# ZYM-PKU/UDiffText

Measured on AMD Instinct MI355X. Metric: 512x512 50-step denoised images/sec (UDiffText hot path: conditioner + 50 CFG Euler steps + VAE decode), higher is better.
Workload: dtype bf16; 1 GPU; 512x512, 50 Euler/DDIM(eta 0) steps, CFG 5.0, 9-char labels, noise_iters 0; global batch 4 per step sharded over 1 GPU(s) = 4 images per GPU in micro-batches of 4: every UNet call runs ONE batch of 4 (8 samples with CFG); 3 such batch(es) in flight per GPU on separate launch streams; BASELINE.json configs[1]; global_batch=4, weights=synthetic (name-keyed recipe), 1361.2 M parameters, launch=hipGraph replay of the sampler steps, in_flight=3, batches_per_unet_call=1

## Files before the change

udifftext_amd/csrc/gemm.hip:

```cpp
#include "common.h"
#include <stdio.h>
#include <stdlib.h>
#include <string.h>
#include <atomic>
#include <cmath>

hipError_t udt_lean_launch_gemm(int cfg, const void* lparams, int smem, int G, int geglu, int ln, hipStream_t s);
hipError_t udt_lean_launch_conv3(const void* c3params, hipStream_t s);

namespace {
#include "tile_common.h"

struct GemmParams {
  const uint16_t* a;
  const uint16_t* a2;
  const uint16_t* w;
  const uint16_t* zero;
  const float* bias;
  const uint16_t* res;
  const float* rowvec;
  void* out;
  const float* colscale;
  const float* in_scsh;
  float* colstats;
// ... 821 lines not shown
  t.G = round_workgroups(units);
  int nb = g_n_block.load(std::memory_order_relaxed);
  if (nb <= 0) nb = (t.tiles_m <= 8) ? t.tiles_n : 8;
  if (nb > t.tiles_n) nb = t.tiles_n;
  t.n_block = nb;
  return true;
}

size_t lean_workspace(const LeanPlan& t) {
  return t.splitk > 1 ? G8_HEADER_BYTES + (size_t)t.tiles * t.splitk * t.bm * t.bn * sizeof(float) : 0;
}

std::atomic<int> g_lean_conv{-1};
std::atomic<int> g_wide_conv{-2};
int wide_conv_mode() {
  int v = g_wide_conv.load(std::memory_order_relaxed);
  if (v == -2) {
    const char* e = getenv("UDT_WIDE_CONV");
    v = e ? atoi(e) : -1;
    g_wide_conv.store(v, std::memory_order_relaxed);
  }
  return v;
}
#ifdef UDT_MEASURE
std::atomic<int> g_lconv_dbg{0};
#endif

std::atomic<int> g_wide_lanes_eff{-2};
double wide_lanes_eff() {
  int v = g_wide_lanes_eff.load(std::memory_order_relaxed);
  if (v == -2) {
    const char* e = getenv("UDT_WIDE_LANES_EFF");
    v = e ? atoi(e) : 70;
    g_wide_lanes_eff.store(v, std::memory_order_relaxed);
  }
  return v / 100.0;
}

int conv_chunk_slices(long long tiles, int slots, int chunks, int knob) {
  long long sk = 1;
  if (tiles <= 1023) {
    if (knob > 1) { sk = knob; if (sk > chunks) sk = chunks; }
    else if (knob < 0 && tiles * 2 <= slots && chunks >= 10) { sk = slots / tiles; if (sk > chunks / 4) sk = chunks / 4; }
    if (sk < 1) sk = 1;
  }
  return (int)sk;
// ... 13 lines not shown
  if (d->N < 128 || d->N % 8 != 0 || d->C1 <= 0 || d->C1 % 64 != 0) return false;
  if (d->upsample != 0 && d->upsample != 1 && d->upsample != 2) return false;
  const bool phase = d->upsample == 2, ups = d->upsample == 1;
  const int nph = phase ? 4 : 1;
  if (d->Hout != (d->Hin << (d->upsample ? 1 : 0)) || d->Wout != (d->Win << (d->upsample ? 1 : 0))) return false;
  if (phase && d->ldw > 0 && d->ldw < 4 * d->C1) return false;
  const int Ht = phase ? d->Hin : d->Hout, Wt = phase ? d->Win : d->Wout;
  c.bn = 128; c.wgm = 2;
  bool wide = false;
  int wide_slots = device_cus();
  {
    const int wm = wide_conv_mode();
    if (wm != 0 && !ups && d->N % 160 == 0 && Wt % 16 == 0 && Ht % 16 == 0) {
      const int cus = device_cus(), share = d->cu_share > 1 ? d->cu_share : 1;
      wide_slots = cus / share > 0 ? cus / share : 1;
      const long long wt = (long long)(d->M / 256) * (d->N / 160);
      const long long sk = conv_chunk_slices(wt, wide_slots, d->C1 / 64, lean_splitk_knob());
      const long long units = wt * sk;
      const long long rounds = (units + cus - 1) / cus;
      const double eff = units > cus ? (double)units / (double)(rounds * cus) : ((double)units * share >= cus ? 1.0 : (double)units * share / cus);
      wide = (wm > 0) || (sk <= 2 && eff >= ((share >= 3 && share_of(d) >= 3) ? wide_lanes_eff() : 0.85));
    }
  }
  if (wide) { c.geo = phase ? 6 : 3; c.tw = 16; c.th = 16; c.bn = 160; c.wgm = 4; }
  else if (Wt % 16 == 0 && Ht % 8 == 0) { c.geo = ups ? 2 : phase ? 4 : 0; c.tw = 16; c.th = 8; }
  else if (!ups && Wt % 8 == 0 && Ht % 8 == 0) { c.geo = phase ? 5 : 1; c.tw = 8; c.th = 8; }
  else return false;
  if (d->ldo % 8 != 0 || (d->residual && d->ldr % 8 != 0)) return false;
  const long long ldw = d->ldw > 0 ? d->ldw : (phase ? 4LL * d->C1 : (long long)d->K);
  if (ldw % 8 != 0) return false;
  c.w_phase = phase ? (d->stride_w > 0 ? d->stride_w : (long long)d->N * ldw) : 0;
  if (phase && (c.w_phase < (long long)d->N * ldw || c.w_phase % 8 != 0)) return false;
  if ((long long)d->M * d->C1 * 2 >= (1LL << 31) || (long long)d->N * ldw * 2 >= (1LL << 31)) return false;
  if ((reinterpret_cast<uintptr_t>(d->out) | reinterpret_cast<uintptr_t>(d->residual) | reinterpret_cast<uintptr_t>(d->bias) |
       reinterpret_cast<uintptr_t>(d->rowvec)) & 15) return false;
  if (d->rowvec && ((d->ld_rowvec > 0 ? d->ld_rowvec : d->N) % 4 != 0)) return false;
  c.dbg = 0;
#ifdef UDT_MEASURE
  c.dbg = g_lconv_dbg.load(std::memory_order_relaxed);
#endif
  c.N = d->N; c.C = d->C1; c.H = d->Hin; c.W = d->Win; c.B = d->M / (d->Hout * d->Wout);
  c.ldw = (int)ldw; c.ldo = d->ldo; c.ldr = d->ldr; c.ldrv = d->ld_rowvec > 0 ? d->ld_rowvec : d->N;
  c.alpha = d->alpha;
  c.tiles_x = Wt / c.tw; c.tiles_y = Ht / c.th;
  c.tiles_m = c.B * c.tiles_x * c.tiles_y;
  c.tiles_n = (d->N + c.bn - 1) / c.bn;
  c.tiles = c.tiles_m * c.tiles_n;
// ... 38 lines not shown
  LeanPlan lt;
  if (lean_plan(d, lt, true)) {
    rows = lt.stats_rows;
    slots = lt.tiles_m * (lt.bm / lt.stats_rows);
    return true;
  }
  return false;
}
}

extern "C" int udt_debug_set(const char* key, int32_t value) {
  if (!key) return UDT_ERR_BAD_ARG;
  if (!strcmp(key, "n_block")) { g_n_block.store(value); return UDT_OK; }
  if (!strcmp(key, "rows_epi")) { g_rows_epi.store(value ? 1 : 0); return UDT_OK; }
  if (!strcmp(key, "lean")) { g_lean.store(value < 0 ? -2 : value); return UDT_OK; }
  if (!strcmp(key, "rowres")) { g_rowres.store(value < 0 ? 1 : (value ? 1 : 0)); return UDT_OK; }
  if (!strcmp(key, "wide_lanes_eff")) { g_wide_lanes_eff.store(value < 0 ? -2 : value); return UDT_OK; }
  if (!strcmp(key, "conv_n4")) { g_conv_n4.store(value < 0 ? -2 : (value ? 1 : 0)); return UDT_OK; }
  if (!strcmp(key, "lean256_lanes")) { g_lean256_lanes.store(value < 0 ? -2 : (value ? 1 : 0)); return UDT_OK; }
  if (!strcmp(key, "lean_splitk")) { g_lean_splitk.store(value); return UDT_OK; }
  if (!strcmp(key, "share_splitk")) { g_share_splitk.store(value < 0 ? -2 : (value ? 1 : 0)); return UDT_OK; }
  if (!strcmp(key, "lean_conv")) { g_lean_conv.store(value < 0 ? -1 : (value ? 1 : 0)); return UDT_OK; }
  if (!strcmp(key, "wide_conv")) { g_wide_conv.store(value < 0 ? -1 : (value ? 1 : 0)); return UDT_OK; }
#ifdef UDT_MEASURE
  if (!strcmp(key, "lconv_dbg")) { g_lconv_dbg.store(value); return UDT_OK; }
  static const struct { const char* k; int bit; } bits[] = {{"no_xchg", 28}, {"no_epi", 27}, {"no_store", 26}, {"no_res", 25},
                                                            {"no_bias", 24}, {"no_fast", 22}};
  for (const auto& b : bits)
    if (!strcmp(key, b.k)) {
      int cur = g_dbg_bits.load();
      g_dbg_bits.store((cur & ~(1 << b.bit)) | (value ? (1 << b.bit) : 0));
      return UDT_OK;
    }
#endif
  return UDT_ERR_BAD_ARG;
}

extern "C" int udt_check_async_error(void* workspace, size_t workspace_bytes, void* stream) {
  if (!workspace || workspace_bytes < G8_HEADER_BYTES) return UDT_ERR_BAD_ARG;
  hipStream_t s = reinterpret_cast<hipStream_t>(stream);
  int err = 0;
  hipError_t e = hipMemcpyAsync(&err, reinterpret_cast<int*>(workspace) + 1023, sizeof(int), hipMemcpyDeviceToHost, s);
  if (e == hipSuccess) e = hipStreamSynchronize(s);
  if (e != hipSuccess) return udt_set_hip_error(e);
  if (err == 0) return UDT_OK;
  e = hipMemsetAsync(workspace, 0, G8_HEADER_BYTES, s);
// ... 215 lines not shown
        udt_prof_tag(profl.rec, tag);
      }
      const bool geglu = (d->flags & UDT_GEMM_GEGLU) != 0, ln = d->ln_colsum != nullptr;
      hipError_t el;
      el = udt_lean_launch_gemm(lt.cfg, &lp, lt.smem, lt.G, geglu ? 1 : 0, ln ? 1 : 0, s);
      if (el != hipSuccess) return udt_set_hip_error(el);
      return UDT_OK;
    }
  }
  if (d->ln_colsum) return UDT_ERR_BAD_ARG;
  {
    lg::C3Params c3;
    if (lean_conv_plan(d, c3, d->colstats != nullptr)) {
      c3.colstats = d->colstats;
      c3.a = p.a; c3.w = p.w; c3.bias = p.bias; c3.res = p.res; c3.rowvec = p.rowvec; c3.out = reinterpret_cast<uint16_t*>(d->out);
      if (c3.splitk > 1) {
        if (!workspace || workspace_bytes < lean_conv_workspace(c3)) return UDT_ERR_WORKSPACE;
        c3.counters = reinterpret_cast<int*>(workspace);
        c3.slabs = reinterpret_cast<float*>(reinterpret_cast<char*>(workspace) + G8_HEADER_BYTES);
      }
      UdtProfScope profc(cls, s);
      if (profc.rec) {
        char tag[96];
        snprintf(tag, sizeof(tag), "%s%s M=%d N=%d K=%d %dx%d tile=%dx%d units=%d splitk=%d nb=%d%s", (c3.geo == 3 || c3.geo == 6) ? "wconv3" : "lconv3",
                 (d->upsample && c3.geo != 6) ? "+up" : "", d->M, d->N, d->K,
                 d->Hin, d->Win, c3.tw, c3.th, c3.tiles * lean_conv_phases(c3) * c3.splitk, c3.splitk, c3.n_block,
                 d->upsample == 2 ? " up4" : "");
        udt_prof_tag(profc.rec, tag);
      }
      const hipError_t ec = udt_lean_launch_conv3(&c3, s);
      if (ec != hipSuccess) return udt_set_hip_error(ec);
      return UDT_OK;
    }
  }
  {
    c3p::CParams cp;
    if (conv3p_geometry(d, cp.geo, d->in_scsh != nullptr)) {
      const TilePlan t3 = plan_tiles3p(d, cp.geo);
      p.tiles_m = t3.tiles_m; p.tiles_n = t3.tiles_n; p.tiles_per_batch = t3.tiles_m * t3.tiles_n;
      {
        const double patch = (double)cp.geo.prows_img * cp.geo.NI * cp.geo.C * 2.0;
        const double wtile = 9.0 * t3.bn * cp.geo.C * 2.0;
        const double S = (double)(t3.tiles < t3.G ? t3.tiles : t3.G) / 8.0;
        int nb = (int)(std::sqrt((S < 1.0 ? 1.0 : S) * patch / wtile) + 0.5);
        if (nb < 1) nb = 1;
        if (nb > t3.tiles_n) nb = t3.tiles_n;
        p.n_block = nb;
      }
      p.n_ktiles = t3.nkt;
// ... 111 lines not shown
```

udifftext_amd/csrc/lean.hip:

```cpp
#include "common.h"
#include <stdio.h>
#include <stdlib.h>
#include <atomic>

namespace {
#include "tile_common.h"
#include "lean_params.h"
#include "lean.h"
#include "wide.h"
#include "rowres.h"

template <int NW, int WGM, int WGN, int TM, int TN, int NST, int TMB = TM>
hipError_t launch_lean(const lg::LParams& lp, int smem, int G, bool geglu, bool ln, hipStream_t s) {
  static AttrOnce once[5];
  const void* fn;
  const bool stats = lp.colstats != nullptr;
  if constexpr (NW == 4 && NST == 2) {
    if (stats) {
      fn = (const void*)lg::lgemm_kernel<NW, WGM, WGN, TM, TN, NST, false, false, TMB, true>;
      hipError_t e = once[4].ensure(fn, smem);
      if (e != hipSuccess) return e;
      void* args[] = {const_cast<lg::LParams*>(&lp)};
      return hipLaunchKernel(fn, dim3(G), dim3(NW * 64), args, smem, s);
    }
// ... 28 lines not shown
  }
  if (geglu) return (ln && emit && !stats) ? launch_lean_mx8_k<true, true, false, true, true>(lp, smem, G, s) : hipErrorInvalidValue;
  if (ln) return stats ? hipErrorInvalidValue
                 : emit ? launch_lean_mx8_k<false, true, false, true, true>(lp, smem, G, s)
                        : launch_lean_mx8_k<false, true, false, true, false>(lp, smem, G, s);
  if (stats) return emit ? hipErrorInvalidValue : launch_lean_mx8_k<false, false, true, true, false>(lp, smem, G, s);
  return emit ? launch_lean_mx8_k<false, false, false, true, true>(lp, smem, G, s) : launch_lean_mx8_k<false, false, false, true, false>(lp, smem, G, s);
}

template <int TW, int TH, bool UPS, bool STATS, bool PHASE>
hipError_t launch_lconv3s(const lg::C3Params& c3, hipStream_t s) {
  static AttrOnce once;
  constexpr int smem = lg::C3Geo<TW, TH, UPS>::SMEM;
  hipError_t e = once.ensure(reinterpret_cast<const void*>(lg::lconv3_kernel<TW, TH, UPS, STATS, PHASE>), smem);
  if (e != hipSuccess) return e;
  hipLaunchKernelGGL((lg::lconv3_kernel<TW, TH, UPS, STATS, PHASE>), dim3(c3.G), dim3(256), smem, s, c3);
  return hipGetLastError();
}
template <int TW, int TH, bool UPS, bool PHASE = false>
hipError_t launch_lconv3(const lg::C3Params& c3, hipStream_t s) {
  return c3.colstats ? launch_lconv3s<TW, TH, UPS, true, PHASE>(c3, s) : launch_lconv3s<TW, TH, UPS, false, PHASE>(c3, s);
}

template <bool STATS, bool PHASE>
hipError_t launch_wconv3s(const lg::C3Params& c3, hipStream_t s) {
  static AttrOnce once;
  constexpr int smem = wd::WGeo::SMEM;
  hipError_t e = once.ensure(reinterpret_cast<const void*>(wd::wconv3_kernel<STATS, PHASE>), smem);
  if (e != hipSuccess) return e;
  hipLaunchKernelGGL((wd::wconv3_kernel<STATS, PHASE>), dim3(c3.G), dim3(256), smem, s, c3);
  return hipGetLastError();
}
template <int KT, bool GEGLU, bool EMIT = false>
hipError_t launch_rowres(const lg::LParams& lp, int G, hipStream_t s) {
  static AttrOnce once;
  constexpr int smem = rr::RGeo<KT, GEGLU>::SMEM;
  hipError_t e = once.ensure(reinterpret_cast<const void*>(rr::rgemm_kernel<KT, GEGLU, EMIT>), smem);
  if (e != hipSuccess) return e;
  hipLaunchKernelGGL((rr::rgemm_kernel<KT, GEGLU, EMIT>), dim3(G), dim3(256), smem, s, lp);
  return hipGetLastError();
}

template <bool PHASE>
hipError_t launch_wconv3(const lg::C3Params& c3, hipStream_t s) {
  return c3.colstats ? launch_wconv3s<true, PHASE>(c3, s) : launch_wconv3s<false, PHASE>(c3, s);
}

}

hipError_t udt_lean_launch_gemm(int cfg, const void* lparams, int smem, int G, int geglu, int ln, hipStream_t s) {
  const lg::LParams& lp = *static_cast<const lg::LParams*>(lparams);
  const bool fp8 = lp.a_scale != nullptr, emit = lp.q8_out != nullptr;
  if (cfg == 7 && emit && !fp8 && !geglu && ln && lp.K == 320) return launch_rowres<5, false, true>(lp, G, s);
  if (fp8 || emit) return cfg == 1 ? launch_lean_mx8(lp, smem, G, geglu != 0, ln != 0, fp8, emit, s) : hipErrorInvalidValue;
  switch (cfg) {
    case 1: return launch_lean<4, 2, 2, 2, 2, 2>(lp, smem, G, geglu != 0, ln != 0, s);
    case 6: return launch_lean<8, 2, 4, 4, 2, 2, 1>(lp, smem, G, geglu != 0, ln != 0, s);
    case 5: return geglu ? hipErrorInvalidValue : launch_lean<4, 4, 1, 1, 5, 2>(lp, smem, G, false, ln != 0, s);
    case 7:
      if (!ln || lp.K != 320) return hipErrorInvalidValue;
      return geglu ? launch_rowres<5, true>(lp, G, s) : launch_rowres<5, false>(lp, G, s);
    default: return hipErrorInvalidValue;
  }
}

hipError_t udt_lean_launch_conv3(const void* c3params, hipStream_t s) {
  const lg::C3Params& c3 = *static_cast<const lg::C3Params*>(c3params);
  return c3.geo == 3 ? launch_wconv3<false>(c3, s) : c3.geo == 6 ? launch_wconv3<true>(c3, s) : c3.geo == 2 ? launch_lconv3<16, 8, true>(c3, s)
// ... 4 lines not shown
```

udifftext_amd/csrc/lean_params.h:

```cpp
#pragma once

namespace lg {

struct LParams {
  const uint16_t* a;
  const uint16_t* a2;
  const uint16_t* w;
  const float* bias;
  const uint16_t* res;
  const float* rowvec;
  const float* ln_s;
  uint16_t* out;
  int M, N, K;
  int lda, ldw, ldo, ldr, ldrv, rows_per_batch;
  float alpha, ln_eps;
  int tiles_m, tiles_n, n_block, tiles;
  int nkt;
  int splitk, kt_per;
  unsigned a_bytes, w_bytes;
  int kt_split, lda2;
  unsigned a2_bytes;
  int G;
  int* counters;
  float* slabs;
// ... 10 lines not shown
  float* rowstat_out;
};

struct C3Params {
  const uint16_t* a;
  const uint16_t* w;
  const float* bias;
  const uint16_t* res;
  const float* rowvec;
  uint16_t* out;
  int N, C;
  int B, H, W;
  int ldw, ldo, ldr, ldrv;
  float alpha;
  int tiles_x, tiles_y, tiles_m, tiles_n, n_block, tiles;
  int chunks, splitk, ch_per;
  unsigned a_bytes, w_bytes;
  int G;
  int* counters;
  float* slabs;
  float* colstats;
  int geo, tw, th;
  int bn, wgm;
  long long w_phase;
  int dbg;
};

}
```

udifftext_amd/csrc/wide.h:

```cpp
#pragma once
#include <type_traits>

namespace wd {

using g8::buf_lds16;
using g8::OOB;
using g8::wait_vm;
using lg::C3Params;
using lg::raw_barrier;
using lg::wait_vm_upto;
using lg::wave_colstats;

struct WGeo {
  static constexpr int TW = 16, TH = 16, NW = 4;
  static constexpr int TM = 2, TN = 5, BN = TN * 32;
  static constexpr int PW = TW + 2, PH = TH + 2, PROWS = PW * PH;
  static constexpr int PIECES = (PROWS + 7) / 8;
  static constexpr int PATCH_BYTES = PIECES * 1024;
  static constexpr int W_BYTES = BN * ROW_BYTES;
  static constexpr int NRING = 3;
  static constexpr int RING = NRING * W_BYTES + 2 * PATCH_BYTES;
  static constexpr int EROW = BN * 4;
  static constexpr int STAGING = NW * 32 * EROW;
  static constexpr int SMEM = RING > STAGING ? RING : STAGING;
  static_assert(SMEM <= 160 * 1024, "one workgroup per CU");
};

template <bool STATS, bool PHASE = false>
__global__ void __launch_bounds__(256, 1) wconv3_kernel(const C3Params p) {
  using G = WGeo;
  constexpr int NT = PHASE ? 4 : 9;
  constexpr int NW = G::NW, TM = G::TM, TN = G::TN, BN = G::BN, PW = G::PW, NR = G::NRING;
  constexpr int WP = (BN / 8) / NW;
  constexpr int PP = (G::PIECES + NW - 1) / NW;
  constexpr int EROW = G::EROW;
  static_assert((BN / 8) % NW == 0, "weight pieces split evenly over the waves");
  extern __shared__ __attribute__((aligned(16))) char smem[];
  char* const wring = smem;
  char* const patches = smem + NR * G::W_BYTES;

  const int tid = threadIdx.x;
  const int wave = __builtin_amdgcn_readfirstlane(tid >> 6);
  const int lane = tid & 63;
  const int l31 = lane & 31;
  const int hi = lane >> 5;
  const int l3 = lane >> 3;
  const int pslot = lane & 7;
  const int row0 = wave * (TM * 32);
  const int swz_w = (l31 >> 1) & 7;
  const int w_frag_row = l31 * ROW_BYTES;

  const int unit = range_index(blockIdx.x, p.G);
  if (unit >= p.tiles * p.splitk * (PHASE ? 4 : 1)) return;
  const int phase = PHASE ? unit / (p.tiles * p.splitk) : 0;
  const int pha = phase >> 1, phb = phase & 1;
  const int ptile = unit / p.splitk;
  const int slice = unit - ptile * p.splitk;
  const int tile = ptile - phase * p.tiles;
  int tile_m, n0;
  {
    const int per_block = p.tiles_m * p.n_block;
    const int blk = tile / per_block;
    const int r = tile - blk * per_block;
    int nbw = p.tiles_n - blk * p.n_block;
    if (nbw > p.n_block) nbw = p.n_block;
    tile_m = r / nbw;
    n0 = (blk * p.n_block + (r - tile_m * nbw)) * BN;
  }
  const int per_img = p.tiles_x * p.tiles_y;
  const int b = tile_m / per_img;
  const int rt = tile_m - b * per_img;
  const int ty = rt / p.tiles_x;
  const int y0 = ty * G::TH, x0 = (rt - ty * p.tiles_x) * G::TW;
  const int c0 = slice * p.ch_per;
  int c1 = c0 + p.ch_per;
  if (c1 > p.chunks) c1 = p.chunks;

  const __amdgpu_buffer_rsrc_t rsrc_a = __builtin_amdgcn_make_buffer_rsrc(const_cast<uint16_t*>(p.a), 0, p.a_bytes, 0x00020000);
  const __amdgpu_buffer_rsrc_t rsrc_w =
      __builtin_amdgcn_make_buffer_rsrc(const_cast<uint16_t*>(p.w) + (PHASE ? (long long)phase * p.w_phase : 0LL), 0, p.w_bytes, 0x00020000);
  auto patch_swz = [](int prow, int yy) { return ((prow - 2 * yy) >> 1) & 7; };
  unsigned w_voff[WP], p_voff[PP];
  int p_piece[PP];
#pragma unroll
  for (int i = 0; i < WP; ++i) {
    const int row = (wave + NW * i) * 8 + l3;
    const int kw = (pslot ^ ((row >> 1) & 7)) * 8;
    const int n = n0 + row;
    w_voff[i] = (n < p.N) ? (unsigned)(((long long)n * p.ldw + kw) * 2) : OOB;
  }
#pragma unroll
  for (int i = 0; i < PP; ++i) {
    int idx = wave + NW * i;
    while (idx >= G::PIECES) idx -= NW;
    p_piece[i] = idx;
    const int prow = idx * 8 + l3;
    const int yy = prow / PW;
    const int xx = prow - yy * PW;
    const int gy = y0 + yy - 1, gx = x0 + xx - 1;
    const bool ok = (prow < G::PROWS) && ((unsigned)gy < (unsigned)p.H) && ((unsigned)gx < (unsigned)p.W);
    const int koff = (pslot ^ patch_swz(prow, yy)) * 8;
    p_voff[i] = ok ? (unsigned)(((((long long)b * p.H + gy) * p.W + gx) * p.C + koff) * 2) : OOB;
  }
  int a_prow[TM], a_py[TM];
#pragma unroll
  for (int tm = 0; tm < TM; ++tm) {
    const int ml = row0 + tm * 32 + l31;
    const int py = ml / G::TW, px = ml - py * G::TW;
    a_py[tm] = PHASE ? py + pha : py;
    a_prow[tm] = PHASE ? (py + pha) * PW + px + phb : py * PW + px;
  }
  auto issue_w = [&](int st, int c, int tap) {
    const int soff = (tap * p.C + c * 64) * 2;
    char* wbuf = wring + st * G::W_BYTES;
#pragma unroll
    for (int i = 0; i < WP; ++i) buf_lds16(rsrc_w, wbuf + (wave + NW * i) * 1024, w_voff[i], soff);
  };
  auto issue_patch = [&](int buf, int c) {
    char* pbuf = patches + buf * G::PATCH_BYTES;
#pragma unroll
    for (int i = 0; i < PP; ++i) buf_lds16(rsrc_a, pbuf + p_piece[i] * 1024, p_voff[i], c * 128);
  };

  f32x16 acc[TM][TN];
#pragma unroll
  for (int i = 0; i < TM; ++i)
#pragma unroll
    for (int j = 0; j < TN; ++j)
#pragma unroll
      for (int r = 0; r < 16; ++r) acc[i][j][r] = 0.f;

  constexpr int PPT = PHASE ? 6 : 2, PTAPS = (PP + PPT - 1) / PPT;
  static_assert(PTAPS <= NT - 2, "the next patch is complete two taps before its chunk starts");
  static_assert(NR - 1 < NT, "the ring's prologue stays inside the first chunk");
  auto issue_patch_part = [&](int buf, int c, int part) {
    char* pbuf = patches + buf * G::PATCH_BYTES;
#pragma unroll
    for (int j = 0; j < PPT; ++j) {
      const int i = part * PPT + j;
      if (i < PP) buf_lds16(rsrc_a, pbuf + p_piece[i] * 1024, p_voff[i], c * 128);
    }
  };
  issue_patch(c0 & 1, c0);
#pragma unroll
  for (int j = 0; j < NR - 1; ++j) issue_w(j, c0, j);
  int st = 0;
  for (int c = c0; c < c1; ++c) {
    const int cn = (c + 1 < c1) ? c + 1 : c;
    const char* pbuf = patches + (c & 1) * G::PATCH_BYTES;
    auto tap_body = [&](auto tap_c) {
      constexpr int tap = decltype(tap_c)::value;
      constexpr auto pcount = [](int t) { const int tt = (t + NT) % NT; return tt < PTAPS ? ((tt + 1) * PPT <= PP ? PPT : PP - tt * PPT) : 0; };
      wait_vm<pcount(tap - 2) + WP + pcount(tap - 1)>();
      raw_barrier();
      const int dy = PHASE ? tap >> 1 : tap / 3, dx = PHASE ? tap & 1 : tap - dy * 3;
      const char* wbuf = wring + st * G::W_BYTES;
      int arow[TM], aswz[TM];
#pragma unroll
      for (int t = 0; t < TM; ++t) {
        const int prow = a_prow[t] + dy * PW + dx;
        arow[t] = prow * ROW_BYTES;
        aswz[t] = patch_swz(prow, a_py[t] + dy);
      }
      bf16x8_t fx[2][TM], fw[2][TN];
      auto read_ks = [&](int ks, int slot2) {
        if (UDT_DBG(p.dbg, 3)) return;
#pragma unroll
        for (int t = 0; t < TM; ++t) fx[slot2][t] = lds_read_frag(pbuf + arow[t] + (((ks * 2 + hi) ^ aswz[t]) << 4));
        const int slot = ((ks * 2 + hi) ^ swz_w) << 4;
#pragma unroll
        for (int t = 0; t < TN; ++t) fw[slot2][t] = lds_read_frag(wbuf + w_frag_row + t * 32 * ROW_BYTES + slot);
      };
      read_ks(0, 0);
#pragma unroll
      for (int ks = 0; ks < 4; ++ks) {
        if (ks + 1 < 4) read_ks(ks + 1, (ks + 1) & 1);
        if (ks == 3) {
          const int ahead = tap + NR - 1;
          int s2 = st + NR - 1;
          if (s2 >= NR) s2 -= NR;
          if (!UDT_DBG(p.dbg, 0)) {
            if (ahead < NT) issue_w(s2, c, ahead);
            else issue_w(s2, cn, ahead - NT);
          }
          if constexpr (tap < PTAPS) {
            if (!UDT_DBG(p.dbg, 1)) issue_patch_part((c + 1) & 1, cn, tap);
          }
        }
        if (UDT_DBG(p.dbg, 2)) {
#pragma unroll
          for (int tm = 0; tm < TM; ++tm) asm volatile("" ::"v"(fx[ks & 1][tm]));
#pragma unroll
          for (int tn = 0; tn < TN; ++tn) asm volatile("" ::"v"(fw[ks & 1][tn]));
        } else {
#pragma unroll
          for (int tm = 0; tm < TM; ++tm)
#pragma unroll
            for (int tn = 0; tn < TN; ++tn) acc[tm][tn] = mfma32(fw[ks & 1][tn], fx[ks & 1][tm], acc[tm][tn]);
        }
      }
      __builtin_amdgcn_sched_group_barrier(0x100, TM + TN, 0);
#pragma unroll
      for (int ks = 0; ks < 3; ++ks) {
#pragma unroll
        for (int i = 0; i < TM + TN; ++i) {
          __builtin_amdgcn_sched_group_barrier(0x008, 1, 0);
          __builtin_amdgcn_sched_group_barrier(0x100, 1, 0);
        }
        __builtin_amdgcn_sched_group_barrier(0x008, TM * TN - (TM + TN), 0);
      }
      constexpr int NV = WP + pcount(tap), NVI = NV < TM * TN ? NV : TM * TN;
#pragma unroll
      for (int i = 0; i < NVI; ++i) {
        __builtin_amdgcn_sched_group_barrier(0x008, 1, 0);
        __builtin_amdgcn_sched_group_barrier(0x020, 1, 0);
      }
      if constexpr (NV > NVI) __builtin_amdgcn_sched_group_barrier(0x020, NV - NVI, 0);
      else __builtin_amdgcn_sched_group_barrier(0x008, TM * TN - NV, 0);
      st = (st + 1 == NR) ? 0 : st + 1;
    };
    tap_body(std::integral_constant<int, 0>{}); tap_body(std::integral_constant<int, 1>{}); tap_body(std::integral_constant<int, 2>{});
    tap_body(std::integral_constant<int, 3>{});
    if constexpr (!PHASE) {
      tap_body(std::integral_constant<int, 4>{}); tap_body(std::integral_constant<int, 5>{});
      tap_body(std::integral_constant<int, 6>{}); tap_body(std::integral_constant<int, 7>{}); tap_body(std::integral_constant<int, 8>{});
    }
  }
  constexpr int CPR = TN * 4;
  constexpr int RPI = 64 / CPR;
  constexpr int NIT = (32 + RPI - 1) / RPI;
  const int rl = lane / CPR;
  const int c8 = lane - rl * CPR;
  const int n = n0 + c8 * 8;
  const bool col_ok = (rl < RPI) && (n < p.N);
  long long mrow[TM][NIT];
  bool rok[TM][NIT];
  u32x4 rv[TM][NIT];
#pragma unroll
  for (int tm = 0; tm < TM; ++tm)
#pragma unroll
    for (int i = 0; i < NIT; ++i) {
      const int row = i * RPI + rl;
      rok[tm][i] = col_ok && row < 32;
      const int ml = row0 + tm * 32 + (row < 32 ? row : 0);
      const int py = ml / G::TW, px = ml - py * G::TW;
      mrow[tm][i] = PHASE ? ((long long)b * (2 * p.H) + (2 * (y0 + py) + pha)) * (2 * p.W) + (2 * (x0 + px) + phb)
                          : ((long long)b * p.H + (y0 + py)) * p.W + (x0 + px);
      u32x4 z = {0u, 0u, 0u, 0u};
      rv[tm][i] = z;
      if (p.res && rok[tm][i]) rv[tm][i] = *reinterpret_cast<const u32x4*>(p.res + mrow[tm][i] * p.ldr + n);
    }
  wait_vm<0>();
  raw_barrier();

  if (p.splitk > 1) {
    f32x4* slab = reinterpret_cast<f32x4*>(p.slabs + (long long)unit * (G::TW * G::TH * BN));
#pragma unroll
    for (int tm = 0; tm < TM; ++tm)
#pragma unroll
      for (int tn = 0; tn < TN; ++tn)
#pragma unroll
        for (int q = 0; q < 4; ++q) {
          f32x4 v = {acc[tm][tn][q * 4 + 0], acc[tm][tn][q * 4 + 1], acc[tm][tn][q * 4 + 2], acc[tm][tn][q * 4 + 3]};
          store16_sc1(slab + ((tm * TN + tn) * 4 + q) * 256 + tid, v);
        }
    asm volatile("s_waitcnt vmcnt(0)" ::: "memory");
    __syncthreads();
    int* const bcast = reinterpret_cast<int*>(smem);
    if (tid == 0) {
      const int t = __hip_atomic_fetch_add(p.counters + ptile, 1, __ATOMIC_RELAXED, __HIP_MEMORY_SCOPE_AGENT);
      const int last = (t == p.splitk - 1) ? 1 : 0;
      if (last) {
        __builtin_amdgcn_fence(__ATOMIC_ACQUIRE, "agent");
        __hip_atomic_store(p.counters + ptile, 0, __ATOMIC_RELAXED, __HIP_MEMORY_SCOPE_AGENT);
      }
      *bcast = last;
    }
    __syncthreads();
    const bool last = *bcast != 0;
    __syncthreads();
    if (!last) return;
#pragma unroll
    for (int i = 0; i < TM; ++i)
#pragma unroll
      for (int j = 0; j < TN; ++j)
#pragma unroll
        for (int r = 0; r < 16; ++r) acc[i][j][r] = 0.f;
    for (int s = 0; s < p.splitk; ++s) {
      const f32x4* sl = reinterpret_cast<const f32x4*>(p.slabs + ((long long)ptile * p.splitk + s) * (G::TW * G::TH * BN));
#pragma unroll
      for (int tm = 0; tm < TM; ++tm)
#pragma unroll
        for (int tn = 0; tn < TN; ++tn)
#pragma unroll
          for (int q = 0; q < 4; ++q) {
            const f32x4 v = sl[((tm * TN + tn) * 4 + q) * 256 + tid];
#pragma unroll
            for (int r = 0; r < 4; ++r) acc[tm][tn][q * 4 + r] += v[r];
          }
    }
  }

  char* const wl = smem + wave * (32 * EROW);
  f32x4 b0 = {0.f, 0.f, 0.f, 0.f}, b1 = b0;
  if (col_ok) {
    if (p.bias) {
      b0 = *reinterpret_cast<const f32x4*>(p.bias + n);
      b1 = *reinterpret_cast<const f32x4*>(p.bias + n + 4);
    }
    if (p.rowvec) {
      const float* rvp = p.rowvec + (long long)b * p.ldrv + n;
      const f32x4 r0 = *reinterpret_cast<const f32x4*>(rvp), r1 = *reinterpret_cast<const f32x4*>(rvp + 4);
#pragma unroll
      for (int j = 0; j < 4; ++j) b0[j] += r0[j], b1[j] += r1[j];
    }
  }
  float cs[8], cq[8];
#pragma unroll
  for (int j = 0; j < 8; ++j) cs[j] = cq[j] = 0.f;
#pragma unroll
  for (int tm = 0; tm < TM; ++tm) {
    {
      const int row = l31;
#pragma unroll
      for (int tn = 0; tn < TN; ++tn)
#pragma unroll
        for (int q = 0; q < 4; ++q) {
          const int chunk = (tn * 8 + q * 2 + hi) ^ (row & 7);
          f32x4 v = {acc[tm][tn][q * 4 + 0], acc[tm][tn][q * 4 + 1], acc[tm][tn][q * 4 + 2], acc[tm][tn][q * 4 + 3]};
          *reinterpret_cast<f32x4*>(wl + row * EROW + chunk * 16) = v;
        }
    }
#pragma unroll
    for (int i = 0; i < NIT; ++i) {
      const int row = i * RPI + rl;
      const int rr = row < 32 ? row : 0;
      const char* rp = wl + rr * EROW;
      const int sw = rr & 7;
      const f32x4 v0 = *reinterpret_cast<const f32x4*>(rp + (((2 * c8) ^ sw) << 4));
      const f32x4 v1 = *reinterpret_cast<const f32x4*>(rp + (((2 * c8 + 1) ^ sw) << 4));
      float o[8];
#pragma unroll
      for (int j = 0; j < 4; ++j) {
        o[j] = v0[j] * p.alpha + b0[j];
        o[4 + j] = v1[j] * p.alpha + b1[j];
      }
      if (p.res) {
#pragma unroll
        for (int j = 0; j < 4; ++j) {
          o[2 * j] += bf16_lo(rv[tm][i][j]);
          o[2 * j + 1] += bf16_hi(rv[tm][i][j]);
        }
      }
      if (rok[tm][i]) {
        u32x4 pk = {pack_bf16x2(o[0], o[1]), pack_bf16x2(o[2], o[3]), pack_bf16x2(o[4], o[5]), pack_bf16x2(o[6], o[7])};
        *reinterpret_cast<u32x4*>(p.out + mrow[tm][i] * p.ldo + n) = pk;
        if constexpr (STATS) {
#pragma unroll
          for (int j = 0; j < 4; ++j) {
            const float a = bf16_lo(pk[j]), bb = bf16_hi(pk[j]);
            cs[2 * j] += a; cq[2 * j] += a * a;
            cs[2 * j + 1] += bb; cq[2 * j + 1] += bb * bb;
          }
        }
      }
    }
  }
  if constexpr (STATS) {
    const int slot = (PHASE ? (b * 4 + phase) * per_img + rt : tile_m) * NW + wave;
    wave_colstats<CPR, RPI>(wl, lane, cs, cq, p.colstats + ((long long)slot * p.N + n) * 2, col_ok);
  }
}

}
```

Baseline: 10.65 images/s.

## Split wide conv3 K-steps across paired wave groups with 512-thread workgroups

Adds an 8-wave (PAIR) variant of the wide 3x3 conv kernel, enabled by default. Two groups of four waves each take half of the K-substeps per tap and half of the weight and patch loads. The partial accumulators are then reduced through LDS before the first group runs the epilogue. This doubles the waves per CU to hide LDS and MFMA latency in a one-workgroup-per-CU kernel. The cost is an extra LDS reduction with barriers, an idle half during the epilogue, and residual loads moved later into the epilogue.

```diff
diff --git a/udifftext_amd/csrc/gemm.hip b/udifftext_amd/csrc/gemm.hip
--- a/udifftext_amd/csrc/gemm.hip
+++ b/udifftext_amd/csrc/gemm.hip
@@ -867,6 +867,12 @@
   }
   return v;
 }
+constexpr int WIDE_WAVES_DEFAULT = 8;
+std::atomic<int> g_wide_waves{-1};
+int wide_waves() {
+  const int v = g_wide_waves.load(std::memory_order_relaxed);
+  return (v == 4 || v == 8) ? v : WIDE_WAVES_DEFAULT;
+}
 #ifdef UDT_MEASURE
 std::atomic<int> g_lconv_dbg{0};
 #endif
@@ -926,7 +932,8 @@
       wide = (wm > 0) || (sk <= 2 && eff >= ((share >= 3 && share_of(d) >= 3) ? wide_lanes_eff() : 0.85));
     }
   }
-  if (wide) { c.geo = phase ? 6 : 3; c.tw = 16; c.th = 16; c.bn = 160; c.wgm = 4; }
+  c.wwaves = 0;
+  if (wide) { c.geo = phase ? 6 : 3; c.tw = 16; c.th = 16; c.bn = 160; c.wgm = 4; c.wwaves = wide_waves(); }
   else if (Wt % 16 == 0 && Ht % 8 == 0) { c.geo = ups ? 2 : phase ? 4 : 0; c.tw = 16; c.th = 8; }
   else if (!ups && Wt % 8 == 0 && Ht % 8 == 0) { c.geo = phase ? 5 : 1; c.tw = 8; c.th = 8; }
   else return false;
@@ -1011,6 +1018,11 @@
   if (!strcmp(key, "share_splitk")) { g_share_splitk.store(value < 0 ? -2 : (value ? 1 : 0)); return UDT_OK; }
   if (!strcmp(key, "lean_conv")) { g_lean_conv.store(value < 0 ? -1 : (value ? 1 : 0)); return UDT_OK; }
   if (!strcmp(key, "wide_conv")) { g_wide_conv.store(value < 0 ? -1 : (value ? 1 : 0)); return UDT_OK; }
+  if (!strcmp(key, "wide_waves")) {
+    if (value >= 0 && value != 4 && value != 8) return UDT_ERR_BAD_ARG;
+    g_wide_waves.store(value < 0 ? -1 : value);
+    return UDT_OK;
+  }
 #ifdef UDT_MEASURE
   if (!strcmp(key, "lconv_dbg")) { g_lconv_dbg.store(value); return UDT_OK; }
   static const struct { const char* k; int bit; } bits[] = {{"no_xchg", 28}, {"no_epi", 27}, {"no_store", 26}, {"no_res", 25},
@@ -1272,9 +1284,10 @@
       UdtProfScope profc(cls, s);
       if (profc.rec) {
         char tag[96];
-        snprintf(tag, sizeof(tag), "%s%s M=%d N=%d K=%d %dx%d tile=%dx%d units=%d splitk=%d nb=%d%s", (c3.geo == 3 || c3.geo == 6) ? "wconv3" : "lconv3",
+        snprintf(tag, sizeof(tag), "%s%s M=%d N=%d K=%d %dx%d tile=%dx%d units=%d splitk=%d nb=%d%s%s", (c3.geo == 3 || c3.geo == 6) ? "wconv3" : "lconv3",
                  (d->upsample && c3.geo != 6) ? "+up" : "", d->M, d->N, d->K,
                  d->Hin, d->Win, c3.tw, c3.th, c3.tiles * lean_conv_phases(c3) * c3.splitk, c3.splitk, c3.n_block,
+                 (c3.wwaves == 0 || c3.wwaves == WIDE_WAVES_DEFAULT) ? "" : (c3.wwaves == 8 ? " waves=8" : " waves=4"),
                  d->upsample == 2 ? " up4" : "");
         udt_prof_tag(profc.rec, tag);
       }
diff --git a/udifftext_amd/csrc/lean.hip b/udifftext_amd/csrc/lean.hip
--- a/udifftext_amd/csrc/lean.hip
+++ b/udifftext_amd/csrc/lean.hip
@@ -74,13 +74,13 @@
   return c3.colstats ? launch_lconv3s<TW, TH, UPS, true, PHASE>(c3, s) : launch_lconv3s<TW, TH, UPS, false, PHASE>(c3, s);
 }
 
-template <bool STATS, bool PHASE>
+template <bool STATS, bool PHASE, bool PAIR>
 hipError_t launch_wconv3s(const lg::C3Params& c3, hipStream_t s) {
   static AttrOnce once;
   constexpr int smem = wd::WGeo::SMEM;
-  hipError_t e = once.ensure(reinterpret_cast<const void*>(wd::wconv3_kernel<STATS, PHASE>), smem);
+  hipError_t e = once.ensure(reinterpret_cast<const void*>(wd::wconv3_kernel<STATS, PHASE, PAIR>), smem);
   if (e != hipSuccess) return e;
-  hipLaunchKernelGGL((wd::wconv3_kernel<STATS, PHASE>), dim3(c3.G), dim3(256), smem, s, c3);
+  hipLaunchKernelGGL((wd::wconv3_kernel<STATS, PHASE, PAIR>), dim3(c3.G), dim3(PAIR ? 512 : 256), smem, s, c3);
   return hipGetLastError();
 }
 template <int KT, bool GEGLU, bool EMIT = false>
@@ -95,7 +95,8 @@
 
 template <bool PHASE>
 hipError_t launch_wconv3(const lg::C3Params& c3, hipStream_t s) {
-  return c3.colstats ? launch_wconv3s<true, PHASE>(c3, s) : launch_wconv3s<false, PHASE>(c3, s);
+  if (c3.wwaves == 8) return c3.colstats ? launch_wconv3s<true, PHASE, true>(c3, s) : launch_wconv3s<false, PHASE, true>(c3, s);
+  return c3.colstats ? launch_wconv3s<true, PHASE, false>(c3, s) : launch_wconv3s<false, PHASE, false>(c3, s);
 }
 
 }
diff --git a/udifftext_amd/csrc/lean_params.h b/udifftext_amd/csrc/lean_params.h
--- a/udifftext_amd/csrc/lean_params.h
+++ b/udifftext_amd/csrc/lean_params.h
@@ -56,6 +56,7 @@
   float* colstats;
   int geo, tw, th;
   int bn, wgm;
+  int wwaves;
   long long w_phase;
   int dbg;
 };
diff --git a/udifftext_amd/csrc/wide.h b/udifftext_amd/csrc/wide.h
--- a/udifftext_amd/csrc/wide.h
+++ b/udifftext_amd/csrc/wide.h
@@ -26,21 +26,22 @@
   static_assert(SMEM <= 160 * 1024, "one workgroup per CU");
 };
 
-template <bool STATS, bool PHASE = false>
-__global__ void __launch_bounds__(256, 1) wconv3_kernel(const C3Params p) {
+template <bool STATS, bool PHASE = false, bool PAIR = false>
+__global__ void __launch_bounds__(PAIR ? 512 : 256, 1) wconv3_kernel(const C3Params p) {
   using G = WGeo;
   constexpr int NT = PHASE ? 4 : 9;
   constexpr int NW = G::NW, TM = G::TM, TN = G::TN, BN = G::BN, PW = G::PW, NR = G::NRING;
-  constexpr int WP = (BN / 8) / NW;
-  constexpr int PP = (G::PIECES + NW - 1) / NW;
+  constexpr int KS = PAIR ? 2 : 4;
   constexpr int EROW = G::EROW;
-  static_assert((BN / 8) % NW == 0, "weight pieces split evenly over the waves");
+  static_assert((BN / 8) % NW == 0, "weight pieces split evenly over the pixel blocks");
   extern __shared__ __attribute__((aligned(16))) char smem[];
   char* const wring = smem;
   char* const patches = smem + NR * G::W_BYTES;
 
   const int tid = threadIdx.x;
-  const int wave = __builtin_amdgcn_readfirstlane(tid >> 6);
+  const int wave8 = __builtin_amdgcn_readfirstlane(tid >> 6);
+  const int wave = PAIR ? (wave8 & (NW - 1)) : wave8;
+  const int half = PAIR ? (wave8 >> 2) : 0;
   const int lane = tid & 63;
   const int l31 = lane & 31;
   const int hi = lane >> 5;
@@ -80,28 +81,6 @@
   const __amdgpu_buffer_rsrc_t rsrc_w =
       __builtin_amdgcn_make_buffer_rsrc(const_cast<uint16_t*>(p.w) + (PHASE ? (long long)phase * p.w_phase : 0LL), 0, p.w_bytes, 0x00020000);
   auto patch_swz = [](int prow, int yy) { return ((prow - 2 * yy) >> 1) & 7; };
-  unsigned w_voff[WP], p_voff[PP];
-  int p_piece[PP];
-#pragma unroll
-  for (int i = 0; i < WP; ++i) {
-    const int row = (wave + NW * i) * 8 + l3;
-    const int kw = (pslot ^ ((row >> 1) & 7)) * 8;
-    const int n = n0 + row;
-    w_voff[i] = (n < p.N) ? (unsigned)(((long long)n * p.ldw + kw) * 2) : OOB;
-  }
-#pragma unroll
-  for (int i = 0; i < PP; ++i) {
-    int idx = wave + NW * i;
-    while (idx >= G::PIECES) idx -= NW;
-    p_piece[i] = idx;
-    const int prow = idx * 8 + l3;
-    const int yy = prow / PW;
-    const int xx = prow - yy * PW;
-    const int gy = y0 + yy - 1, gx = x0 + xx - 1;
-    const bool ok = (prow < G::PROWS) && ((unsigned)gy < (unsigned)p.H) && ((unsigned)gx < (unsigned)p.W);
-    const int koff = (pslot ^ patch_swz(prow, yy)) * 8;
-    p_voff[i] = ok ? (unsigned)(((((long long)b * p.H + gy) * p.W + gx) * p.C + koff) * 2) : OOB;
-  }
   int a_prow[TM], a_py[TM];
 #pragma unroll
   for (int tm = 0; tm < TM; ++tm) {
@@ -110,121 +89,159 @@
     a_py[tm] = PHASE ? py + pha : py;
     a_prow[tm] = PHASE ? (py + pha) * PW + px + phb : py * PW + px;
   }
-  auto issue_w = [&](int st, int c, int tap) {
-    const int soff = (tap * p.C + c * 64) * 2;
-    char* wbuf = wring + st * G::W_BYTES;
-#pragma unroll
-    for (int i = 0; i < WP; ++i) buf_lds16(rsrc_w, wbuf + (wave + NW * i) * 1024, w_voff[i], soff);
+
+  f32x16 acc[TM][TN];
+#pragma unroll
+  for (int i = 0; i < TM; ++i)
+#pragma unroll
+    for (int j = 0; j < TN; ++j)
+#pragma unroll
+      for (int r = 0; r < 16; ++r) acc[i][j][r] = 0.f;
+
+  auto main_loop = [&](auto half_c) {
+    constexpr int HF = decltype(half_c)::value;
+    constexpr int WP = PAIR ? (HF ? 2 : 3) : (BN / 8) / NW;
+    constexpr int W0 = PAIR ? (HF ? 3 * NW : 0) : 0;
+    constexpr int PP = PAIR ? (HF ? 7 : 4) : (G::PIECES + NW - 1) / NW;
+    constexpr int P0 = PAIR ? (HF ? 4 * NW : 0) : 0;
+    constexpr int KB = HF * 2;
+    static_assert(!PAIR || (3 + 2) * NW == BN / 8, "the two halves cover the weight tile");
+    static_assert(!PAIR || (4 + 7) * NW >= G::PIECES, "the two halves cover the patch");
+    unsigned w_voff[WP], p_voff[PP];
+    int p_piece[PP];
+#pragma unroll
+    for (int i = 0; i < WP; ++i) {
+      const int row = (W0 + wave + NW * i) * 8 + l3;
+      const int kw = (pslot ^ ((row >> 1) & 7)) * 8;
+      const int n = n0 + row;
+      w_voff[i] = (n < p.N) ? (unsigned)(((long long)n * p.ldw + kw) * 2) : OOB;
+    }
+#pragma unroll
+    for (int i = 0; i < PP; ++i) {
+      int idx = P0 + wave + NW * i;
+      while (idx >= G::PIECES) idx -= NW;
+      p_piece[i] = idx;
+      const int prow = idx * 8 + l3;
+      const int yy = prow / PW;
+      const int xx = prow - yy * PW;
+      const int gy = y0 + yy - 1, gx = x0 + xx - 1;
+      const bool ok = (prow < G::PROWS) && ((unsigned)gy < (unsigned)p.H) && ((unsigned)gx < (unsigned)p.W);
+      const int koff = (pslot ^ patch_swz(prow, yy)) * 8;
+      p_voff[i] = ok ? (unsigned)(((((long long)b * p.H + gy) * p.W + gx) * p.C + koff) * 2) : OOB;
+    }
+    auto issue_w = [&](int st, int c, int tap) {
+      const int soff = (tap * p.C + c * 64) * 2;
+      char* wbuf = wring + st * G::W_BYTES;
+#pragma unroll
+      for (int i = 0; i < WP; ++i) buf_lds16(rsrc_w, wbuf + (W0 + wave + NW * i) * 1024, w_voff[i], soff);
+    };
+    auto issue_patch = [&](int buf, int c) {
+      char* pbuf = patches + buf * G::PATCH_BYTES;
+#pragma unroll
+      for (int i = 0; i < PP; ++i) buf_lds16(rsrc_a, pbuf + p_piece[i] * 1024, p_voff[i], c * 128);
+    };
+    constexpr int PPT = PHASE ? (PAIR ? (HF ? 5 : 2) : 6) : 2, PTAPS = (PP + PPT - 1) / PPT;
+    static_assert(PTAPS <= NT - 2, "the next patch is complete two taps before its chunk starts");
+    static_assert(NR - 1 < NT, "the ring's prologue stays inside the first chunk");
+    auto issue_patch_part = [&](int buf, int c, int part) {
+      char* pbuf = patches + buf * G::PATCH_BYTES;
+#pragma unroll
+      for (int j = 0; j < PPT; ++j) {
+        const int i = part * PPT + j;
+        if (i < PP) buf_lds16(rsrc_a, pbuf + p_piece[i] * 1024, p_voff[i], c * 128);
+      }
+    };
+    issue_patch(c0 & 1, c0);
+#pragma unroll
+    for (int j = 0; j < NR - 1; ++j) issue_w(j, c0, j);
+    int st = 0;
+    for (int c = c0; c < c1; ++c) {
+      const int cn = (c + 1 < c1) ? c + 1 : c;
+      const char* pbuf = patches + (c & 1) * G::PATCH_BYTES;
+      auto tap_body = [&](auto tap_c) {
+        constexpr int tap = decltype(tap_c)::value;
+        constexpr auto pcount = [](int t) { const int tt = (t + NT) % NT; return tt < PTAPS ? ((tt + 1) * PPT <= PP ? PPT : PP - tt * PPT) : 0; };
+        wait_vm<pcount(tap - 2) + WP + pcount(tap - 1)>();
+        raw_barrier();
+        const int dy = PHASE ? tap >> 1 : tap / 3, dx = PHASE ? tap & 1 : tap - dy * 3;
+        const char* wbuf = wring + st * G::W_BYTES;
+        int arow[TM], aswz[TM];
+#pragma unroll
+        for (int t = 0; t < TM; ++t) {
+          const int prow = a_prow[t] + dy * PW + dx;
+          arow[t] = prow * ROW_BYTES;
+          aswz[t] = patch_swz(prow, a_py[t] + dy);
+        }
+        bf16x8_t fx[2][TM], fw[2][TN];
+        auto read_ks = [&](int ks, int slot2) {
+          if (UDT_DBG(p.dbg, 3)) return;
+#pragma unroll
+          for (int t = 0; t < TM; ++t) fx[slot2][t] = lds_read_frag(pbuf + arow[t] + (((ks * 2 + hi) ^ aswz[t]) << 4));
+          const int slot = ((ks * 2 + hi) ^ swz_w) << 4;
+#pragma unroll
+          for (int t = 0; t < TN; ++t) fw[slot2][t] = lds_read_frag(wbuf + w_frag_row + t * 32 * ROW_BYTES + slot);
+        };
+        read_ks(KB, 0);
+#pragma unroll
+        for (int ks = 0; ks < KS; ++ks) {
+          if (ks + 1 < KS) read_ks(KB + ks + 1, (ks + 1) & 1);
+          if (ks == KS - 1) {
+            const int ahead = tap + NR - 1;
+            int s2 = st + NR - 1;
+            if (s2 >= NR) s2 -= NR;
+            if (!UDT_DBG(p.dbg, 0)) {
+              if (ahead < NT) issue_w(s2, c, ahead);
+              else issue_w(s2, cn, ahead - NT);
+            }
+            if constexpr (tap < PTAPS) {
+              if (!UDT_DBG(p.dbg, 1)) issue_patch_part((c + 1) & 1, cn, tap);
+            }
+          }
+          if (UDT_DBG(p.dbg, 2)) {
+#pragma unroll
+            for (int tm = 0; tm < TM; ++tm) asm volatile("" ::"v"(fx[ks & 1][tm]));
+#pragma unroll
+            for (int tn = 0; tn < TN; ++tn) asm volatile("" ::"v"(fw[ks & 1][tn]));
+          } else {
+#pragma unroll
+            for (int tm = 0; tm < TM; ++tm)
+#pragma unroll
+              for (int tn = 0; tn < TN; ++tn) acc[tm][tn] = mfma32(fw[ks & 1][tn], fx[ks & 1][tm], acc[tm][tn]);
+          }
+        }
+        __builtin_amdgcn_sched_group_barrier(0x100, TM + TN, 0);
+#pragma unroll
+        for (int ks = 0; ks < KS - 1; ++ks) {
+#pragma unroll
+          for (int i = 0; i < TM + TN; ++i) {
+            __builtin_amdgcn_sched_group_barrier(0x008, 1, 0);
+            __builtin_amdgcn_sched_group_barrier(0x100, 1, 0);
+          }
+          __builtin_amdgcn_sched_group_barrier(0x008, TM * TN - (TM + TN), 0);
+        }
+        constexpr int NV = WP + pcount(tap), NVI = NV < TM * TN ? NV : TM * TN;
+#pragma unroll
+        for (int i = 0; i < NVI; ++i) {
+          __builtin_amdgcn_sched_group_barrier(0x008, 1, 0);
+          __builtin_amdgcn_sched_group_barrier(0x020, 1, 0);
+        }
+        if constexpr (NV > NVI) __builtin_amdgcn_sched_group_barrier(0x020, NV - NVI, 0);
+        else __builtin_amdgcn_sched_group_barrier(0x008, TM * TN - NV, 0);
+        st = (st + 1 == NR) ? 0 : st + 1;
+      };
+      tap_body(std::integral_constant<int, 0>{}); tap_body(std::integral_constant<int, 1>{}); tap_body(std::integral_constant<int, 2>{});
+      tap_body(std::integral_constant<int, 3>{});
+      if constexpr (!PHASE) {
+        tap_body(std::integral_constant<int, 4>{}); tap_body(std::integral_constant<int, 5>{});
+        tap_body(std::integral_constant<int, 6>{}); tap_body(std::integral_constant<int, 7>{}); tap_body(std::integral_constant<int, 8>{});
+      }
+    }
   };
-  auto issue_patch = [&](int buf, int c) {
-    char* pbuf = patches + buf * G::PATCH_BYTES;
-#pragma unroll
-    for (int i = 0; i < PP; ++i) buf_lds16(rsrc_a, pbuf + p_piece[i] * 1024, p_voff[i], c * 128);
-  };
-
-  f32x16 acc[TM][TN];
-#pragma unroll
-  for (int i = 0; i < TM; ++i)
-#pragma unroll
-    for (int j = 0; j < TN; ++j)
-#pragma unroll
-      for (int r = 0; r < 16; ++r) acc[i][j][r] = 0.f;
-
-  constexpr int PPT = PHASE ? 6 : 2, PTAPS = (PP + PPT - 1) / PPT;
-  static_assert(PTAPS <= NT - 2, "the next patch is complete two taps before its chunk starts");
-  static_assert(NR - 1 < NT, "the ring's prologue stays inside the first chunk");
-  auto issue_patch_part = [&](int buf, int c, int part) {
-    char* pbuf = patches + buf * G::PATCH_BYTES;
-#pragma unroll
-    for (int j = 0; j < PPT; ++j) {
-      const int i = part * PPT + j;
-      if (i < PP) buf_lds16(rsrc_a, pbuf + p_piece[i] * 1024, p_voff[i], c * 128);
-    }
-  };
-  issue_patch(c0 & 1, c0);
-#pragma unroll
-  for (int j = 0; j < NR - 1; ++j) issue_w(j, c0, j);
-  int st = 0;
-  for (int c = c0; c < c1; ++c) {
-    const int cn = (c + 1 < c1) ? c + 1 : c;
-    const char* pbuf = patches + (c & 1) * G::PATCH_BYTES;
-    auto tap_body = [&](auto tap_c) {
-      constexpr int tap = decltype(tap_c)::value;
-      constexpr auto pcount = [](int t) { const int tt = (t + NT) % NT; return tt < PTAPS ? ((tt + 1) * PPT <= PP ? PPT : PP - tt * PPT) : 0; };
-      wait_vm<pcount(tap - 2) + WP + pcount(tap - 1)>();
-      raw_barrier();
-      const int dy = PHASE ? tap >> 1 : tap / 3, dx = PHASE ? tap & 1 : tap - dy * 3;
-      const char* wbuf = wring + st * G::W_BYTES;
-      int arow[TM], aswz[TM];
-#pragma unroll
-      for (int t = 0; t < TM; ++t) {
-        const int prow = a_prow[t] + dy * PW + dx;
-        arow[t] = prow * ROW_BYTES;
-        aswz[t] = patch_swz(prow, a_py[t] + dy);
-      }
-      bf16x8_t fx[2][TM], fw[2][TN];
-      auto read_ks = [&](int ks, int slot2) {
-        if (UDT_DBG(p.dbg, 3)) return;
-#pragma unroll
-        for (int t = 0; t < TM; ++t) fx[slot2][t] = lds_read_frag(pbuf + arow[t] + (((ks * 2 + hi) ^ aswz[t]) << 4));
-        const int slot = ((ks * 2 + hi) ^ swz_w) << 4;
-#pragma unroll
-        for (int t = 0; t < TN; ++t) fw[slot2][t] = lds_read_frag(wbuf + w_frag_row + t * 32 * ROW_BYTES + slot);
-      };
-      read_ks(0, 0);
-#pragma unroll
-      for (int ks = 0; ks < 4; ++ks) {
-        if (ks + 1 < 4) read_ks(ks + 1, (ks + 1) & 1);
-        if (ks == 3) {
-          const int ahead = tap + NR - 1;
-          int s2 = st + NR - 1;
-          if (s2 >= NR) s2 -= NR;
-          if (!UDT_DBG(p.dbg, 0)) {
-            if (ahead < NT) issue_w(s2, c, ahead);
-            else issue_w(s2, cn, ahead - NT);
-          }
-          if constexpr (tap < PTAPS) {
-            if (!UDT_DBG(p.dbg, 1)) issue_patch_part((c + 1) & 1, cn, tap);
-          }
-        }
-        if (UDT_DBG(p.dbg, 2)) {
-#pragma unroll
-          for (int tm = 0; tm < TM; ++tm) asm volatile("" ::"v"(fx[ks & 1][tm]));
-#pragma unroll
-          for (int tn = 0; tn < TN; ++tn) asm volatile("" ::"v"(fw[ks & 1][tn]));
-        } else {
-#pragma unroll
-          for (int tm = 0; tm < TM; ++tm)
-#pragma unroll
-            for (int tn = 0; tn < TN; ++tn) acc[tm][tn] = mfma32(fw[ks & 1][tn], fx[ks & 1][tm], acc[tm][tn]);
-        }
-      }
-      __builtin_amdgcn_sched_group_barrier(0x100, TM + TN, 0);
-#pragma unroll
-      for (int ks = 0; ks < 3; ++ks) {
-#pragma unroll
-        for (int i = 0; i < TM + TN; ++i) {
-          __builtin_amdgcn_sched_group_barrier(0x008, 1, 0);
-          __builtin_amdgcn_sched_group_barrier(0x100, 1, 0);
-        }
-        __builtin_amdgcn_sched_group_barrier(0x008, TM * TN - (TM + TN), 0);
-      }
-      constexpr int NV = WP + pcount(tap), NVI = NV < TM * TN ? NV : TM * TN;
-#pragma unroll
-      for (int i = 0; i < NVI; ++i) {
-        __builtin_amdgcn_sched_group_barrier(0x008, 1, 0);
-        __builtin_amdgcn_sched_group_barrier(0x020, 1, 0);
-      }
-      if constexpr (NV > NVI) __builtin_amdgcn_sched_group_barrier(0x020, NV - NVI, 0);
-      else __builtin_amdgcn_sched_group_barrier(0x008, TM * TN - NV, 0);
-      st = (st + 1 == NR) ? 0 : st + 1;
-    };
-    tap_body(std::integral_constant<int, 0>{}); tap_body(std::integral_constant<int, 1>{}); tap_body(std::integral_constant<int, 2>{});
-    tap_body(std::integral_constant<int, 3>{});
-    if constexpr (!PHASE) {
-      tap_body(std::integral_constant<int, 4>{}); tap_body(std::integral_constant<int, 5>{});
-      tap_body(std::integral_constant<int, 6>{}); tap_body(std::integral_constant<int, 7>{}); tap_body(std::integral_constant<int, 8>{});
-    }
+  if constexpr (PAIR) {
+    if (half) main_loop(std::integral_constant<int, 1>{});
+    else main_loop(std::integral_constant<int, 0>{});
+  } else {
+    main_loop(std::integral_constant<int, 0>{});
   }
   constexpr int CPR = TN * 4;
   constexpr int RPI = 64 / CPR;
@@ -233,37 +250,74 @@
   const int c8 = lane - rl * CPR;
   const int n = n0 + c8 * 8;
   const bool col_ok = (rl < RPI) && (n < p.N);
-  long long mrow[TM][NIT];
-  bool rok[TM][NIT];
-  u32x4 rv[TM][NIT];
-#pragma unroll
-  for (int tm = 0; tm < TM; ++tm)
+  auto rok_of = [&](int i) { return col_ok && i * RPI + rl < 32; };
+  auto mrow_of = [&](int tm, int i) -> long long {
+    const int row = i * RPI + rl;
+    const int ml = row0 + tm * 32 + (row < 32 ? row : 0);
+    const int py = ml / G::TW, px = ml - py * G::TW;
+    return PHASE ? ((long long)b * (2 * p.H) + (2 * (y0 + py) + pha)) * (2 * p.W) + (2 * (x0 + px) + phb)
+                 : ((long long)b * p.H + (y0 + py)) * p.W + (x0 + px);
+  };
+  constexpr int RVP = PAIR ? 1 : TM;
+  u32x4 rv[RVP][NIT];
+  auto fetch_res = [&](int tm) {
 #pragma unroll
     for (int i = 0; i < NIT; ++i) {
-      const int row = i * RPI + rl;
-      rok[tm][i] = col_ok && row < 32;
-      const int ml = row0 + tm * 32 + (row < 32 ? row : 0);
-      const int py = ml / G::TW, px = ml - py * G::TW;
-      mrow[tm][i] = PHASE ? ((long long)b * (2 * p.H) + (2 * (y0 + py) + pha)) * (2 * p.W) + (2 * (x0 + px) + phb)
-                          : ((long long)b * p.H + (y0 + py)) * p.W + (x0 + px);
       u32x4 z = {0u, 0u, 0u, 0u};
-      rv[tm][i] = z;
-      if (p.res && rok[tm][i]) rv[tm][i] = *reinterpret_cast<const u32x4*>(p.res + mrow[tm][i] * p.ldr + n);
-    }
+      rv[tm % RVP][i] = z;
+      if (p.res && rok_of(i)) rv[tm % RVP][i] = *reinterpret_cast<const u32x4*>(p.res + mrow_of(tm, i) * p.ldr + n);
+    }
+  };
+  if constexpr (!PAIR) {
+#pragma unroll
+    for (int tm = 0; tm < TM; ++tm) fetch_res(tm);
+  }
   wait_vm<0>();
   raw_barrier();
 
+  if constexpr (PAIR) {
+    f32x4* const mg = reinterpret_cast<f32x4*>(smem) + (wave * 64 + lane);
+#pragma unroll
+    for (int tm = 0; tm < TM; ++tm) {
+      if (tm) raw_barrier();
+      if (half) {
+#pragma unroll
+        for (int tn = 0; tn < TN; ++tn)
+#pragma unroll
+          for (int q = 0; q < 4; ++q) {
+            f32x4 v = {acc[tm][tn][q * 4 + 0], acc[tm][tn][q * 4 + 1], acc[tm][tn][q * 4 + 2], acc[tm][tn][q * 4 + 3]};
+            mg[(tn * 4 + q) * (NW * 64)] = v;
+          }
+      }
+      raw_barrier();
+      if (!half) {
+#pragma unroll
+        for (int tn = 0; tn < TN; ++tn)
+#pragma unroll
+          for (int q = 0; q < 4; ++q) {
+            const f32x4 v = mg[(tn * 4 + q) * (NW * 64)];
+#pragma unroll
+            for (int r = 0; r < 4; ++r) acc[tm][tn][q * 4 + r] += v[r];
+          }
+      }
+    }
+    raw_barrier();
+  }
+  const bool owner = !PAIR || half == 0;
+
   if (p.splitk > 1) {
     f32x4* slab = reinterpret_cast<f32x4*>(p.slabs + (long long)unit * (G::TW * G::TH * BN));
-#pragma unroll
-    for (int tm = 0; tm < TM; ++tm)
-#pragma unroll
-      for (int tn = 0; tn < TN; ++tn)
-#pragma unroll
-        for (int q = 0; q < 4; ++q) {
-          f32x4 v = {acc[tm][tn][q * 4 + 0], acc[tm][tn][q * 4 + 1], acc[tm][tn][q * 4 + 2], acc[tm][tn][q * 4 + 3]};
-          store16_sc1(slab + ((tm * TN + tn) * 4 + q) * 256 + tid, v);
-        }
+    if (owner) {
+#pragma unroll
+      for (int tm = 0; tm < TM; ++tm)
+#pragma unroll
+        for (int tn = 0; tn < TN; ++tn)
+#pragma unroll
+          for (int q = 0; q < 4; ++q) {
+            f32x4 v = {acc[tm][tn][q * 4 + 0], acc[tm][tn][q * 4 + 1], acc[tm][tn][q * 4 + 2], acc[tm][tn][q * 4 + 3]};
+            store16_sc1(slab + ((tm * TN + tn) * 4 + q) * 256 + tid, v);
+          }
+    }
     asm volatile("s_waitcnt vmcnt(0)" ::: "memory");
     __syncthreads();
     int* const bcast = reinterpret_cast<int*>(smem);
@@ -279,7 +333,7 @@
     __syncthreads();
     const bool last = *bcast != 0;
     __syncthreads();
-    if (!last) return;
+    if (!last || !owner) return;
 #pragma unroll
     for (int i = 0; i < TM; ++i)
 #pragma unroll
@@ -300,6 +354,7 @@
           }
     }
   }
+  if (!owner) return;
 
   char* const wl = smem + wave * (32 * EROW);
   f32x4 b0 = {0.f, 0.f, 0.f, 0.f}, b1 = b0;
@@ -331,6 +386,7 @@
           *reinterpret_cast<f32x4*>(wl + row * EROW + chunk * 16) = v;
         }
     }
+    if constexpr (PAIR) fetch_res(tm);
 #pragma unroll
     for (int i = 0; i < NIT; ++i) {
       const int row = i * RPI + rl;
@@ -348,13 +404,13 @@
       if (p.res) {
 #pragma unroll
         for (int j = 0; j < 4; ++j) {
-          o[2 * j] += bf16_lo(rv[tm][i][j]);
-          o[2 * j + 1] += bf16_hi(rv[tm][i][j]);
-        }
-      }
-      if (rok[tm][i]) {
+          o[2 * j] += bf16_lo(rv[tm % RVP][i][j]);
+          o[2 * j + 1] += bf16_hi(rv[tm % RVP][i][j]);
+        }
+      }
+      if (rok_of(i)) {
         u32x4 pk = {pack_bf16x2(o[0], o[1]), pack_bf16x2(o[2], o[3]), pack_bf16x2(o[4], o[5]), pack_bf16x2(o[6], o[7])};
-        *reinterpret_cast<u32x4*>(p.out + mrow[tm][i] * p.ldo + n) = pk;
+        *reinterpret_cast<u32x4*>(p.out + mrow_of(tm, i) * p.ldo + n) = pk;
         if constexpr (STATS) {
 #pragma unroll
           for (int j = 0; j < 4; ++j) {
```

After: 10.75 images/s, median of 6. No clear change (+1.0%).
